# scroll-tech/zkevm-circuits

Hardware: AMD Instinct MI355X
Metric: SuperCircuit-shape proof-gen wall-clock (s) at k = 20 (lower is better)
Workload: dtype u32x8 limbs (254-bit modular integer, Montgomery)

## Files before the change

### zkevm-circuits_amd/csrc/msm.hip

```cpp
#include <chrono>
#include <climits>
#include <cmath>

#include "ctx.hpp"
#include "ec29.hip.hpp"
#include "host_fq.hpp"

namespace zk {

constexpr int MSM_MAX_C = 16;
constexpr uint32_t NEG_BIT = 0x80000000u;

struct MsmPlan {
    int c;
    int W;
    uint32_t B;
    int top_shift = 0;
};

struct MsmCol { const Fr* scalars; G1Xyzz* out; };

static MsmPlan make_plan(size_t n) {
    int lg = 0;
    while ((1ull << (lg + 1)) <= n) ++lg;
// ... 141 lines not shown
    uint32_t carry = 0;
#pragma unroll
    for (int w = 0; w < W; ++w) {
        const int bit = w * C, limb = bit >> 5, sh = bit & 31;
        uint32_t d = limb < 8 ? (s.l[limb < 8 ? limb : 7] >> sh) : 0u;
        if (sh + C > 32 && limb + 1 < 8) d |= s.l[limb + 1 < 8 ? limb + 1 : 7] << (32 - sh);
        d = (d & mask) + carry;
        if (w == W - 1) d <<= top_shift;
        if (d > half) { carry = 1; const uint32_t mag = (1u << C) - d; code[w] = mag ? (NEG_BIT | (mag - 1)) : CODE_ZERO; }
        else { carry = 0; code[w] = d ? (d - 1) : CODE_ZERO; }
    }
}
__device__ __forceinline__ uint32_t lds_take(uint32_t* lds, uint32_t slot, bool active) {
    const uint64_t act = __ballot(active);
    if (!active) return 0;
    const uint32_t lane = threadIdx.x & 63u;
    const uint32_t lead = __shfl(slot, (int)__builtin_ctzll(act));
    const uint64_t same = __ballot(slot == lead);
    if (slot == lead) {
        const uint32_t rank = (uint32_t)__popcll(same & ((1ull << lane) - 1ull));
        uint32_t pos = 0;
        if (rank == 0) pos = atomicAdd(&lds[slot], (uint32_t)__popcll(same));
        return __shfl(pos, (int)__builtin_ctzll(same)) + rank;
    }
    return atomicAdd(&lds[slot], 1u);
}
template <int C, bool SCATTER, bool LOWPART = false>
__device__ __forceinline__ void partition_body(const Fr* __restrict__ scalars, uint64_t n, int range_bits, uint32_t* __restrict__ hist, const uint32_t* __restrict__ hist_off,
                                               uint64_t* __restrict__ entries, uint64_t tab_stride, int top_shift, uint32_t bin_base, uint32_t set_mask, uint32_t nwg, uint32_t g, uint32_t* lds) {
    constexpr int W = (256 + C - 1) / C;
    const uint32_t nbins = (set_mask + 1u) << (C - 1 - range_bits);
    for (uint32_t t = threadIdx.x; t < nbins; t += blockDim.x) lds[t] = SCATTER ? hist_off[(uint64_t)(bin_base + t) * nwg + g] : 0u;
    __syncthreads();
    const uint64_t chunk = (n + nwg - 1) / nwg;
    const uint64_t lo = min(n, (uint64_t)g * chunk), hi = min(n, lo + chunk);
    const uint32_t rmask = (1u << range_bits) - 1u;
    for (uint64_t base = lo; base < hi; base += blockDim.x) {
        const uint64_t i = base + threadIdx.x;
        const bool live = i < hi;
        uint32_t code[W];
        if (live) recode_wide<C>(from_mont(ldg(scalars + i)), code, top_shift);
        else {
#pragma unroll
            for (int w = 0; w < W; ++w) code[w] = CODE_ZERO;
        }
#pragma unroll
        for (int w = 0; w < W; ++w) {
            const bool nz = code[w] != CODE_ZERO;
            if (!__ballot(nz)) continue;
            uint32_t part, local;
            if (LOWPART) {
                const int PB = C - 1 - range_bits;
                const uint32_t b = code[w] & 0x3FFFFFu;
                part = ((((uint32_t)w & set_mask)) << PB) | (b & ((1u << PB) - 1u));
                local = b >> PB;
            } else {
                const uint32_t bucket = (code[w] & 0x3FFFFFu) | (((uint32_t)w & set_mask) << (C - 1));
                part = bucket >> range_bits;
                local = bucket & rmask;
            }
            const uint32_t pos = lds_take(lds, part, nz);
            if (SCATTER && nz) entries[pos] = ((uint64_t)local << 32) | (uint64_t)((uint32_t)((uint64_t)w * tab_stride + i) | (code[w] & NEG_BIT));
        }
    }
    if (!SCATTER) {
        __syncthreads();
        for (uint32_t t = threadIdx.x; t < nbins; t += blockDim.x) hist[(uint64_t)(bin_base + t) * nwg + g] = lds[t];
    }
}
template <int C, bool SCATTER>
__global__ void __launch_bounds__(256) k_msm_m_partition(const Fr* __restrict__ scalars_arg, uint64_t n, int range_bits, uint32_t* __restrict__ hist, const uint32_t* __restrict__ hist_off,
                                                          uint64_t* __restrict__ entries, uint64_t tab_stride, int top_shift, const MsmCol* __restrict__ cols = nullptr, const uint32_t* __restrict__ ctr = nullptr) {
    const Fr* __restrict__ scalars = cols ? cols[*ctr].scalars : scalars_arg;
    __shared__ uint32_t lds[MSM_M_MAX_BINS];
    partition_body<C, SCATTER>(scalars, n, range_bits, hist, hist_off, entries, tab_stride, top_shift, 0u, 0u, gridDim.x, blockIdx.x, lds);
}
constexpr int GM_MAX_COLS = 16;
struct GmCols { const Fr* p[GM_MAX_COLS]; };
template <int C, bool SCATTER>
__global__ void __launch_bounds__(256) k_msm_gm_partition(GmCols cols, uint64_t n, int range_bits, uint32_t* __restrict__ hist, const uint32_t* __restrict__ hist_off,
                                                           uint64_t* __restrict__ entries, uint64_t tab_stride, uint32_t bins_per_col, uint32_t set_mask) {
    __shared__ uint32_t lds[MSM_M_MAX_BINS];
    partition_body<C, SCATTER, true>(cols.p[blockIdx.y], n, range_bits, hist, hist_off, entries, tab_stride, 0, blockIdx.y * bins_per_col, set_mask, gridDim.x, blockIdx.x, lds);
}
constexpr uint32_t MSM_M_SCHUNK = 1024;
template <int C>
__global__ void __launch_bounds__(1024) k_msm_m_scatter_staged(const Fr* __restrict__ scalars_arg, uint64_t n, int range_bits, const uint32_t* __restrict__ hist_off,
                                                               uint64_t* __restrict__ entries, uint64_t tab_stride, int top_shift, const MsmCol* __restrict__ cols = nullptr, const uint32_t* __restrict__ ctr = nullptr) {
    constexpr int W = (256 + C - 1) / C;
    const Fr* __restrict__ scalars = cols ? cols[*ctr].scalars : scalars_arg;
    extern __shared__ __attribute__((aligned(16))) uint32_t sm[];
    uint32_t* cnt = sm;
    uint32_t* gdelta = sm + MSM_M_MAX_BINS;
    uint32_t* wtot = gdelta + MSM_M_MAX_BINS;
    uint64_t* stage = reinterpret_cast<uint64_t*>(wtot + 16);
    uint16_t* pid = reinterpret_cast<uint16_t*>(stage + (size_t)MSM_M_SCHUNK * W);
    const uint32_t nbins = 1u << (C - 1 - range_bits), nwg = gridDim.x, g = blockIdx.x;
    const uint32_t rmask = (1u << range_bits) - 1u;
    cnt[threadIdx.x] = 0u;
    __syncthreads();
    const uint64_t chunk = (n + nwg - 1) / nwg;
    const uint64_t i = min(n, (uint64_t)g * chunk) + threadIdx.x;
    const bool live = threadIdx.x < chunk && i < min(n, ((uint64_t)g + 1) * chunk);
    uint32_t code[W], rank[W];
    if (live) recode_wide<C>(from_mont(ldg(scalars + i)), code, top_shift);
    else {
#pragma unroll
        for (int w = 0; w < W; ++w) code[w] = CODE_ZERO;
    }
#pragma unroll
    for (int w = 0; w < W; ++w) {
        const bool nz = code[w] != CODE_ZERO;
        rank[w] = 0;
        if (!__ballot(nz)) continue;
        rank[w] = lds_take(cnt, (code[w] & 0x3FFFFFu) >> range_bits, nz);
    }
    __syncthreads();
    {
        const uint32_t c0 = threadIdx.x < nbins ? cnt[threadIdx.x] : 0u;
        const uint32_t lane = threadIdx.x & 63u, wave = threadIdx.x >> 6;
        uint32_t incl = c0;
#pragma unroll
        for (int off = 1; off < 64; off <<= 1) { const uint32_t o = __shfl_up(incl, off); if (lane >= (uint32_t)off) incl += o; }
        if (lane == 63) wtot[wave] = incl;
        __syncthreads();
        uint32_t wbase = 0;
        for (uint32_t w = 0; w < wave; ++w) wbase += wtot[w];
        const uint32_t ex = wbase + incl - c0;
        if (threadIdx.x < nbins) {
            cnt[threadIdx.x] = ex;
            gdelta[threadIdx.x] = hist_off[(uint64_t)threadIdx.x * nwg + g] - ex;
        }
    }
    __syncthreads();
    uint32_t total = 0;
    for (uint32_t w = 0; w < 16; ++w) total += wtot[w];
#pragma unroll
    for (int w = 0; w < W; ++w) {
        if (code[w] == CODE_ZERO) continue;
        const uint32_t bucket = code[w] & 0x3FFFFFu, part = bucket >> range_bits;
        const uint32_t pos = cnt[part] + rank[w];
        stage[pos] = ((uint64_t)(bucket & rmask) << 32) | (uint64_t)((uint32_t)((uint64_t)w * tab_stride + i) | (code[w] & NEG_BIT));
        pid[pos] = (uint16_t)part;
    }
    __syncthreads();
    for (uint32_t e = threadIdx.x; e < total; e += blockDim.x) entries[gdelta[pid[e]] + e] = stage[e];
}
static size_t scatter_staged_lds(int W) { return (size_t)(2 * MSM_M_MAX_BINS + 16) * 4 + (size_t)MSM_M_SCHUNK * W * 10; }
template <bool SCATTER>
__global__ void __launch_bounds__(1024) k_msm_m_bin(const uint64_t* __restrict__ entries, const uint32_t* __restrict__ hist_off, uint32_t nwg, int range_bits,
                                                    uint32_t* __restrict__ counts, const uint32_t* __restrict__ offsets, uint32_t* __restrict__ idx) {
    __shared__ uint32_t lds[1 << MSM_RANGE_MAX_BITS];
    const uint32_t nbins_ = gridDim.x / MSM_SLICES;
    uint32_t bin, sl;
    if ((nbins_ & 7u) == 0) {
        const uint32_t xcd = blockIdx.x & 7u, slot = blockIdx.x >> 3;
        sl = slot % MSM_SLICES;
        bin = (slot / MSM_SLICES) * 8u + xcd;
    } else {
        bin = blockIdx.x / MSM_SLICES;
        sl = blockIdx.x % MSM_SLICES;
    }
    const uint32_t range = 1u << range_bits;
    const uint64_t gbase = (uint64_t)bin << range_bits;
    for (uint32_t t = threadIdx.x; t < range; t += blockDim.x) lds[t] = SCATTER ? offsets[(gbase + t) * MSM_SLICES + sl] : 0u;
    __syncthreads();
// ... 570 lines not shown
    __syncthreads();
}
template <bool LAST>
__global__ void __launch_bounds__(256) k_wsum_level(const G1Xyzz29* __restrict__ in, uint32_t count, G1Xyzz29* __restrict__ S_out, G1Xyzz29* __restrict__ Tpart, G1Xyzz29* __restrict__ U_out) {
    __shared__ G1Xyzz29 sh[LAST ? 512 : 256];
    const uint32_t g = blockIdx.x * 256 + threadIdx.x, groups = (count + WS_G - 1) / WS_G;
    G1Xyzz29 acc = identity29(), run = identity29();
    if (g < groups) {
        const uint32_t b0 = g * WS_G, b1 = min(b0 + WS_G, count);
        for (uint32_t b = b1; b-- > b0;) { acc = add29pt(acc, run); run = add29pt(run, ldg29(in + b)); }
        if (LAST) { if (b0) acc = add29pt(acc, mul_small(run, b0)); }
        else stg29(S_out + g, run);
    }
    if (LAST) {
        block_sum29x2(acc, run, sh);
        if (threadIdx.x == 0) { stg29(Tpart + blockIdx.x, acc); stg29(U_out, run); }
    } else {
        const G1Xyzz29 t = block_sum29(acc, sh);
        if (threadIdx.x == 0) stg29(Tpart + blockIdx.x, t);
    }
}
struct WsumPlan { int levels; uint32_t off[WS_MAX_LEVELS], cnt[WS_MAX_LEVELS]; };
__global__ void __launch_bounds__(256) k_wsum_final(const G1Xyzz29* __restrict__ Tpart, WsumPlan pl, const G1Xyzz29* __restrict__ U, G1Xyzz* __restrict__ out) {
    __shared__ G1Xyzz29 A[WS_MAX_LEVELS];
    const uint32_t wave = threadIdx.x >> 6, lane = threadIdx.x & 63u;
    for (int lv = (int)wave; lv < pl.levels; lv += 4) {
        G1Xyzz29 a = identity29();
        for (uint32_t i = lane; i < pl.cnt[lv]; i += 64) a = add29pt(a, ldg29(Tpart + pl.off[lv] + i));
        for (int off = 32; off > 0; off >>= 1) a = add29pt(a, shfl_down_pt(a, off));
        if (lane == 0) A[lv] = a;
    }
    __syncthreads();
    if (threadIdx.x == 0) {
        G1Xyzz29 T = A[pl.levels - 1];
        for (int lv = pl.levels - 2; lv >= 0; --lv) {
            for (int d = 1; d < WS_G; d <<= 1) T = dbl29pt(T);
            T = add29pt(T, A[lv]);
        }
        stg(out, to_std_xyzz(add29pt(T, ldg29(U))));
    }
}
static int wsum_enqueue(zk_ctx* ctx, hipStream_t st, const G1Xyzz29* buckets, uint32_t nb, G1Xyzz29* scratch, G1Xyzz* out) {
    WsumPlan pl;
    pl.levels = 0;
    uint32_t tparts = 0, count = nb;
    uint32_t t_total = 1;
    for (uint32_t c_ = nb; ; ) {
        const uint32_t groups = (c_ + WS_G - 1) / WS_G;
        t_total += c_ <= WS_LAST_MAX ? 1 : (groups + 255) / 256;
        if (c_ <= WS_LAST_MAX) break;
        c_ = groups;
    }
    G1Xyzz29* U = scratch;
    G1Xyzz29* Tpart = scratch + 1;
    G1Xyzz29* S = scratch + t_total;
    const G1Xyzz29* in = buckets;
    while (count > WS_LAST_MAX) {
        if (pl.levels >= WS_MAX_LEVELS - 1) return ctx->fail(ZK_ERR_UNSUPPORTED, "bucket reduction: too many levels");
        const uint32_t groups = (count + WS_G - 1) / WS_G, blocks = (groups + 255) / 256;
        pl.off[pl.levels] = tparts; pl.cnt[pl.levels] = blocks;
        hipLaunchKernelGGL((k_wsum_level<false>), dim3(blocks), dim3(256), 0, st, in, count, S, Tpart + tparts, (G1Xyzz29*)nullptr);
        tparts += blocks;
        ++pl.levels;
        in = S;
        S += groups;
        count = groups;
    }
    pl.off[pl.levels] = tparts; pl.cnt[pl.levels] = 1;
    hipLaunchKernelGGL((k_wsum_level<true>), dim3(1), dim3(256), 0, st, in, count, (G1Xyzz29*)nullptr, Tpart + tparts, U);
    ++pl.levels;
    hipLaunchKernelGGL(k_wsum_final, dim3(1), dim3(256), 0, st, (const G1Xyzz29*)Tpart, pl, (const G1Xyzz29*)U, out);
    ZK_CHECK_LAUNCH(ctx);
    return ZK_OK;
}

#define PK_TRY_MSM(expr) do { int rc__ = (expr); if (rc__) return rc__; } while (0)

constexpr int KNOB_UNSET = INT_MIN;
struct MsmKnobs {
    int c, top_shift;
    int binsort, staged, chunk;
    int pipes, graph;
    int narrow, narrow_group, narrow_gm, gm_sets;
    double table_gb;
    bool trace;
};
static MsmKnobs read_knobs() {
    auto num = [](const char* name) { const char* e = getenv(name); return e ? atoi(e) : KNOB_UNSET; };
    MsmKnobs k;
    k.c = num("ZK_MSM_C");
    k.top_shift = num("ZK_MSM_TOP_SHIFT");
    k.binsort = num("ZK_MSM_BINSORT");
    k.staged = num("ZK_MSM_STAGED");
    k.chunk = num("ZK_MSM_CHUNK");
    k.pipes = num("ZK_MSM_PIPES");
    k.graph = num("ZK_MSM_GRAPH");
    k.narrow = num("ZK_MSM_NARROW");
    k.narrow_group = num("ZK_MSM_NARROW_GROUP");
    k.narrow_gm = num("ZK_MSM_NARROW_GM");
    k.gm_sets = num("ZK_MSM_GM_SETS");
    const char* gb = getenv("ZK_MSM_TABLE_GB");
    k.table_gb = gb ? atof(gb) : 32.0;
    k.trace = getenv("ZK_MSM_TRACE") != nullptr;
    return k;
}

struct WsCarver {
    uint32_t* base;
    size_t at = 0;
    uint32_t* take(size_t nwords, size_t align_words = 1) {
        at = (at + align_words - 1) / align_words * align_words;
        uint32_t* p = base ? base + at : nullptr;
        at += nwords;
        return p;
    }
};
static inline uint32_t scan_blocks_of(uint32_t cnt) { return (cnt + SCAN_T * SCAN_ITEMS - 1) / (SCAN_T * SCAN_ITEMS); }
constexpr uint32_t MSM_CLEARED_WORDS = SIZE_BINS + 4 + MSM_WFLAGS + TASK_DONE_MAX;
struct SortDims {
    uint32_t nb;
    bool slices;
    uint32_t hist_cnt;
    uint64_t idx_cnt;
    size_t dig_words;
    bool entries;
};
struct SortWs {
    uint32_t *slice_counts, *slice_off, *block_tot_s;
    uint32_t *counts, *offsets, *order, *ntasks, *toff, *block_tot;
    uint32_t *cleared, *size_hist, *nmulti, *wflag;
    uint32_t *hist, *hist_off, *block_tot_h;
    uint32_t* idx;
    uint16_t* dig;
    uint64_t* entries;
    size_t words;
};
static SortWs carve_sort_ws(const SortDims& d, uint32_t* base) {
    WsCarver c{base};
    SortWs w{};
    if (d.slices) {
        w.slice_counts = c.take((size_t)d.nb * MSM_SLICES, 4);
        w.slice_off = c.take((size_t)d.nb * MSM_SLICES + 4, 4);
    }
    w.counts = c.take(d.nb);
    w.cleared = c.take(MSM_CLEARED_WORDS);
    w.size_hist = w.cleared;
    w.nmulti = w.size_hist + SIZE_BINS;
    w.wflag = w.nmulti + 4;
    w.offsets = c.take((size_t)d.nb + 1);
    w.order = c.take(d.nb);
    w.ntasks = c.take(d.nb);
    w.toff = c.take((size_t)d.nb + 1);
    if (d.slices) w.block_tot_s = c.take(scan_blocks_of(d.nb * MSM_SLICES));
    w.block_tot = c.take(scan_blocks_of(d.nb));
    if (d.hist_cnt) {
        w.block_tot_h = c.take(scan_blocks_of(d.hist_cnt));
        w.hist = c.take(d.hist_cnt);
        w.hist_off = c.take((size_t)d.hist_cnt + 1);
    }
    w.idx = c.take(d.idx_cnt);
    if (d.dig_words) w.dig = reinterpret_cast<uint16_t*>(c.take(d.dig_words, 4));
    if (d.entries) w.entries = reinterpret_cast<uint64_t*>(c.take(2 * (size_t)d.idx_cnt, 2));
    w.words = c.at;
    return w;
}

static void scan_blocks(hipStream_t st, const uint32_t* in, uint32_t cnt, uint32_t* out, uint32_t* block_tot, uint32_t* total_out) {
    const uint32_t sb = scan_blocks_of(cnt);
    hipLaunchKernelGGL(k_scan_u32_a, dim3(sb), dim3(SCAN_T), 0, st, in, cnt, out, block_tot);
    hipLaunchKernelGGL(k_scan_u32_b, dim3(1), dim3(SCAN_T), 0, st, block_tot, sb, out, cnt, total_out);
}
static int exclusive_scan(zk_ctx* ctx, hipStream_t st, const uint32_t* in, uint32_t cnt, uint32_t* out, uint32_t* block_tot) {
    scan_blocks(st, in, cnt, out, block_tot, nullptr);
    hipLaunchKernelGGL(k_task_offsets, dim3(scan_blocks_of(cnt)), dim3(SCAN_T), 0, st, cnt, out, (const uint32_t*)block_tot);
    ZK_CHECK_LAUNCH(ctx);
    return ZK_OK;
}
static int slice_scan(zk_ctx* ctx, hipStream_t st, const SortWs& w, uint32_t nb) {
    scan_blocks(st, w.slice_counts, nb * MSM_SLICES, w.slice_off, w.block_tot_s, w.offsets + nb);
    hipLaunchKernelGGL(k_scan_u32_c, dim3(scan_blocks_of(nb * MSM_SLICES)), dim3(SCAN_T), 0, st, (const uint32_t*)w.slice_counts, nb, w.slice_off, (const uint32_t*)w.block_tot_s, w.offsets, w.counts,
                       w.size_hist);
    ZK_CHECK_LAUNCH(ctx);
    return ZK_OK;
// ... 118 lines not shown
    ZK_HIP(ctx, hipEventRecord(ctx->ev_p2[par], ctx->stream2));
    if (stage && it + 1 < count) { int rc = stage(stage_user, it + 1); if (rc) return rc; }
  }
    ZK_HIP(ctx, hipStreamWaitEvent(ctx->stream, ctx->ev_p2[0], 0));
    if (count > 1) ZK_HIP(ctx, hipStreamWaitEvent(ctx->stream, ctx->ev_p2[1], 0));
    std::vector<G1Xyzz> hw((size_t)pl.W * count);
    ZK_HIP(ctx, hipMemcpyAsync(hw.data(), wsum_all, sizeof(G1Xyzz) * pl.W * count, hipMemcpyDeviceToHost, ctx->stream));
    ZK_HIP(ctx, hipStreamSynchronize(ctx->stream));
    for (size_t it = 0; it < count; ++it) host::msm_tail(hw.data() + it * pl.W, red_W, pl.c, h_out + it);
    return ZK_OK;
}
__global__ void __launch_bounds__(1024) k_msm_tails(const Fr* const* __restrict__ scalar_ptrs, const uint8_t* __restrict__ flags, uint64_t n_main, uint32_t tail,
                                                    const G1Affine* __restrict__ table, uint64_t tab_stride, int c, int W, int top_shift, G1Xyzz* __restrict__ out) {
    __shared__ G1Xyzz29 wsum[16];
    const uint32_t col = blockIdx.x;
    G1Xyzz29 acc = identity29();
    if (flags[col] == 1) {
        const Fr* scalars = scalar_ptrs[col];
        for (uint32_t pair = threadIdx.x; pair < tail * (uint32_t)W; pair += blockDim.x) {
            const uint32_t r = pair / (uint32_t)W, w = pair % (uint32_t)W;
            const Fr sc = from_mont(ldg(scalars + n_main + r));
            const int bit = (int)w * c, limb = bit >> 5, sh = bit & 31;
            uint64_t d = limb < 8 ? ((uint64_t)sc.l[limb] >> sh) : 0ull;
            if (limb + 1 < 8) d |= (uint64_t)sc.l[limb + 1] << (32 - sh);
            d &= (1ull << c) - 1;
            int bits = c;
            if ((int)w == W - 1) { d <<= top_shift; bits = c + top_shift; }
            if (d == 0) continue;
            const G1Affine29 base = load_affine29(table + (uint64_t)w * tab_stride + n_main + r);
            G1Xyzz29 t = identity29();
            for (int b = bits - 1; b >= 0; --b) {
                t = dbl29pt(t);
                if ((d >> b) & 1) t = madd29(t, base);
            }
            acc = add29pt(acc, t);
        }
    }
    for (int off = 32; off > 0; off >>= 1) acc = add29pt(acc, shfl_down_pt(acc, off));
    if ((threadIdx.x & 63) == 0) wsum[threadIdx.x >> 6] = acc;
    __syncthreads();
    if (threadIdx.x == 0) {
        G1Xyzz29 s = wsum[0];
        for (uint32_t i = 1; i < blockDim.x / 64; ++i) s = add29pt(s, wsum[i]);
        stg(out + col, to_std_xyzz(s));
    }
}
static MsmPlan make_plan_merged(uint32_t k_srs, const MsmKnobs& kn) {
    int c = (int)k_srs;
    if (c < MSM_M_MIN_C) c = MSM_M_MIN_C;
    if (c > MSM_M_MAX_C) c = MSM_M_MAX_C;
    if (kn.c >= MSM_M_MIN_C && kn.c <= MSM_M_MAX_C) c = kn.c;
    MsmPlan p;
    p.c = c;
    p.W = (256 + c - 1) / c;
    p.B = 1u << (c - 1);
    const int low = c * (p.W - 1);
    uint64_t top_max = 1;
    if (low < 254) {
        uint64_t v = 0;
        for (int b = 0; b < 40 && low + b < 256; ++b) {
            const int bit = low + b;
            const uint32_t limb = bit < 32 ? FrP::M(0) - 1u : FrP::M(bit >> 5);
            v |= (uint64_t)((limb >> (bit & 31)) & 1u) << b;
        }
        top_max = v + 1;
    }
    p.top_shift = 0;
    while (p.top_shift + 1 <= c - 1 && (top_max << (p.top_shift + 1)) <= (1ull << (c - 1))) ++p.top_shift;
    if (kn.top_shift >= 0 && kn.top_shift <= p.top_shift) p.top_shift = kn.top_shift;
    return p;
}
template <bool SCATTER>
static void launch_partition(int c, dim3 grid, hipStream_t st, const Fr* scalars, uint64_t n, int range_bits, uint32_t* hist, const uint32_t* hist_off, uint64_t* entries, uint64_t tab_stride, int top_shift,
                             const MsmCol* cols = nullptr, const uint32_t* ctr = nullptr) {
#define ZK_PART_CASE(C) case C: hipLaunchKernelGGL((k_msm_m_partition<C, SCATTER>), grid, dim3(256), 0, st, scalars, n, range_bits, hist, hist_off, entries, tab_stride, top_shift, cols, ctr); break;
    switch (c) {
        ZK_PART_CASE(8) ZK_PART_CASE(9) ZK_PART_CASE(10) ZK_PART_CASE(11) ZK_PART_CASE(12) ZK_PART_CASE(13) ZK_PART_CASE(14) ZK_PART_CASE(15)
        ZK_PART_CASE(16) ZK_PART_CASE(17) ZK_PART_CASE(18) ZK_PART_CASE(19) ZK_PART_CASE(20) ZK_PART_CASE(21) ZK_PART_CASE(22)
    }
#undef ZK_PART_CASE
}
template <bool SCATTER>
static void launch_gm_partition(int c, dim3 grid, hipStream_t st, const GmCols& cols, uint64_t n, int range_bits, uint32_t* hist, const uint32_t* hist_off, uint64_t* entries, uint64_t tab_stride,
                                uint32_t bins_per_col, uint32_t set_mask) {
#define ZK_GMP_CASE(C) case C: hipLaunchKernelGGL((k_msm_gm_partition<C, SCATTER>), grid, dim3(256), 0, st, cols, n, range_bits, hist, hist_off, entries, tab_stride, bins_per_col, set_mask); break;
    switch (c) {
        ZK_GMP_CASE(8) ZK_GMP_CASE(9) ZK_GMP_CASE(10) ZK_GMP_CASE(11) ZK_GMP_CASE(12) ZK_GMP_CASE(13) ZK_GMP_CASE(14) ZK_GMP_CASE(15) ZK_GMP_CASE(16)
    }
#undef ZK_GMP_CASE
}
static int launch_scatter_staged(zk_ctx* ctx, int c, int W, dim3 grid, const Fr* scalars, uint64_t n, int range_bits, const uint32_t* hist_off, uint64_t* entries, uint64_t tab_stride, int top_shift,
                                 const MsmCol* cols = nullptr, const uint32_t* ctr = nullptr, hipStream_t st = nullptr) {
    const size_t lds = scatter_staged_lds(W);
    if (!st) st = ctx->stream;
#define ZK_SS_CASE(C) case C: \
        if (!(ctx->msm_attr_set & (1u << C))) { ZK_HIP(ctx, hipFuncSetAttribute((const void*)k_msm_m_scatter_staged<C>, hipFuncAttributeMaxDynamicSharedMemorySize, (int)lds)); ctx->msm_attr_set |= 1u << C; } \
        hipLaunchKernelGGL((k_msm_m_scatter_staged<C>), grid, dim3(1024), lds, st, scalars, n, range_bits, hist_off, entries, tab_stride, top_shift, cols, ctr); break;
    switch (c) { ZK_SS_CASE(19) ZK_SS_CASE(20) ZK_SS_CASE(21) ZK_SS_CASE(22) default: return ctx->fail(ZK_ERR_UNSUPPORTED, "staged scatter: window size %d", c); }
#undef ZK_SS_CASE
    ZK_CHECK_LAUNCH(ctx);
    return ZK_OK;
}
static int sort_entries(zk_ctx* ctx, hipStream_t st, const SortWs& w, uint32_t nbins, uint32_t nwg, int range_bits, uint32_t nb, bool binsort) {
    if (binsort) {
        hipLaunchKernelGGL(k_msm_m_binsort, dim3(nbins), dim3(1024), 0, st, (const uint64_t*)w.entries, (const uint32_t*)w.hist_off, nwg, range_bits, nb, w.offsets, w.counts, w.size_hist, w.idx);
        ZK_CHECK_LAUNCH(ctx);
        return task_split(ctx, st, w, nb);
    }
    hipLaunchKernelGGL((k_msm_m_bin<false>), dim3(nbins * MSM_SLICES), dim3(1024), 0, st, (const uint64_t*)w.entries, (const uint32_t*)w.hist_off, nwg, range_bits, w.slice_counts, (const uint32_t*)nullptr, (uint32_t*)nullptr);
    ZK_CHECK_LAUNCH(ctx);
    PK_TRY_MSM(slice_scan(ctx, st, w, nb));
    PK_TRY_MSM(task_split(ctx, st, w, nb));
    hipLaunchKernelGGL((k_msm_m_bin<true>), dim3(nbins * MSM_SLICES), dim3(1024), 0, st, (const uint64_t*)w.entries, (const uint32_t*)w.hist_off, nwg, range_bits, (uint32_t*)nullptr, (const uint32_t*)w.slice_off, w.idx);
    ZK_CHECK_LAUNCH(ctx);
    return ZK_OK;
}
static int sort_partitioned(zk_ctx* ctx, hipStream_t st, const SortWs& w, const MsmPlan& pl, const Fr* scalars, uint64_t n, uint64_t tab_stride, int range_bits, uint32_t nwg, bool staged_scatter, bool binsort,
                            const MsmCol* cols, const uint32_t* ctr) {
    const uint32_t nbins = pl.B >> range_bits;
    ZK_HIP(ctx, hipMemsetAsync(w.cleared, 0, (size_t)MSM_CLEARED_WORDS * 4, st));
    launch_partition<false>(pl.c, dim3(nwg), st, scalars, n, range_bits, w.hist, (const uint32_t*)nullptr, (uint64_t*)nullptr, tab_stride, pl.top_shift, cols, ctr);
    ZK_CHECK_LAUNCH(ctx);
    PK_TRY_MSM(exclusive_scan(ctx, st, w.hist, nbins * nwg, w.hist_off, w.block_tot_h));
    if (staged_scatter) PK_TRY_MSM(launch_scatter_staged(ctx, pl.c, pl.W, dim3(nwg), scalars, n, range_bits, (const uint32_t*)w.hist_off, w.entries, tab_stride, pl.top_shift, cols, ctr, st));
    else launch_partition<true>(pl.c, dim3(nwg), st, scalars, n, range_bits, (uint32_t*)nullptr, (const uint32_t*)w.hist_off, w.entries, tab_stride, pl.top_shift, cols, ctr);
    ZK_CHECK_LAUNCH(ctx);
    return sort_entries(ctx, st, w, nbins, nwg, range_bits, pl.B, binsort);
}
static int sort_gm(zk_ctx* ctx, hipStream_t st, const SortWs& w, const MsmPlan& pl, const Fr* const* scalars, uint32_t cnt, uint64_t n, uint64_t tab_stride, int range_bits, uint32_t nwg, uint32_t bpc, uint32_t sets) {
    const uint32_t nbins = cnt * bpc;
    ZK_HIP(ctx, hipMemsetAsync(w.cleared, 0, (size_t)MSM_CLEARED_WORDS * 4, st));
    GmCols gcols{};
    for (uint32_t j = 0; j < cnt; ++j) gcols.p[j] = scalars[j];
    launch_gm_partition<false>(pl.c, dim3(nwg, cnt), st, gcols, n, range_bits, w.hist, (const uint32_t*)nullptr, (uint64_t*)nullptr, tab_stride, bpc, sets - 1);
    ZK_CHECK_LAUNCH(ctx);
    PK_TRY_MSM(exclusive_scan(ctx, st, w.hist, nbins * nwg, w.hist_off, w.block_tot_h));
    launch_gm_partition<true>(pl.c, dim3(nwg, cnt), st, gcols, n, range_bits, (uint32_t*)nullptr, (const uint32_t*)w.hist_off, w.entries, tab_stride, bpc, sets - 1);
    ZK_CHECK_LAUNCH(ctx);
    return sort_entries(ctx, st, w, nbins, nwg, range_bits, cnt * sets * pl.B, true);
}
static int msm_batch_merged_capped(zk_ctx* ctx, const MsmKnobs& kn, const Fr* const* d_scalar_ptrs, size_t count, const G1Affine* d_table, size_t tab_stride, const MsmPlan& pl,
                                   size_t n, G1Affine* h_out, MsmStageFn stage, void* stage_user, const G1Affine* d_table_n, const MsmPlan* pl_n, const uint8_t* narrow, uint32_t group_cap, uint32_t* smaller_cap) {
    if (count == 0) return ZK_OK;
    if (n == 0) { memset(h_out, 0, sizeof(G1Affine) * count); return ZK_OK; }
    const auto t_batch0 = std::chrono::steady_clock::now();
    bool any_narrow = false;
    if (d_table_n && pl_n && narrow) for (size_t i = 0; i < count; ++i) any_narrow |= narrow[i] == 1;
    if (any_narrow && (uint64_t)n * pl_n->W >= (1ull << 32)) any_narrow = false;
    const uint32_t tail_rows = (any_narrow && ctx->msm_blinded_tail && (size_t)ctx->msm_blinded_tail + 1024 <= n && ctx->msm_blinded_tail <= 256) ? ctx->msm_blinded_tail : 0u;
    const uint64_t n_narrow = (uint64_t)n - tail_rows;
    const MsmPlan pn = any_narrow ? *pl_n : MsmPlan{4, 64, 8};
    uint32_t NG = 1;
    if (any_narrow) {
        NG = std::min<uint32_t>((uint32_t)GM_MAX_COLS, MSM_WFLAGS / (uint32_t)pn.W);
        if (kn.narrow_group >= 1 && kn.narrow_group <= GM_MAX_COLS) NG = std::min<uint32_t>((uint32_t)kn.narrow_group, MSM_WFLAGS / (uint32_t)pn.W);
        if (group_cap && NG > group_cap) NG = group_cap;
        while (NG > 1 && (uint64_t)n * pn.W * NG >= (1ull << 32)) --NG;
        if (NG < 1) NG = 1;
    }
    const uint32_t Wg = (uint32_t)pn.W * NG;
    const uint32_t nbN = Wg * pn.B;
    const uint64_t n_pad = ((uint64_t)n + 16 * MSM_SLICES - 1) & ~(uint64_t)(16 * MSM_SLICES - 1);
    const SortDims dims_N{nbN, true, 0, (uint64_t)n * Wg, (size_t)(n_pad * Wg + 1) / 2 + 4, false};
    const bool gm = any_narrow && pn.c >= MSM_M_MIN_C && pn.c <= 16 && NG <= (uint32_t)GM_MAX_COLS && kn.narrow_gm != 0;
    uint32_t SG = 2;
    if (kn.gm_sets == 1 || kn.gm_sets == 2 || kn.gm_sets == 4) SG = (uint32_t)kn.gm_sets;
    int range_bits_G = pn.c - 1 - 7;
    if (range_bits_G < 0) range_bits_G = 0;
    const uint32_t bpcG = (SG * pn.B) >> range_bits_G;
    const uint32_t perm_G = ((uint32_t)range_bits_G << 8) | (uint32_t)(pn.c - 1 - range_bits_G);
    const uint32_t nwgG = (uint32_t)((n_narrow + MSM_M_CHUNK - 1) / MSM_M_CHUNK);
    const SortDims dims_G{NG * SG * pn.B, false, NG * bpcG * nwgG, (uint64_t)n * pn.W * NG, 0, true};
    const size_t words_N = any_narrow ? std::max(carve_sort_ws(dims_N, nullptr).words, gm ? carve_sort_ws(dims_G, nullptr).words : 0) : 0;
    const uint32_t red_blocks_N = ((pn.B + RED_G_WIDE - 1) / RED_G_WIDE + RED_THREADS - 1) / RED_THREADS;
    const size_t max_tasks_N = (size_t)nbN + std::max(((size_t)n * Wg) / TASK_CAP, (size_t)TASK_TARGET) + 1;
    const size_t npts29_N = any_narrow ? (size_t)nbN + (size_t)red_blocks_N * NG * 4 + max_tasks_N + (size_t)pn.B * NG : 0;
    const uint32_t nb = pl.B;
    const uint64_t max_entries = (uint64_t)n * pl.W;
    if ((uint64_t)pl.W * tab_stride >= (1ull << 31) || max_entries >= (1ull << 32)) return ctx->fail(ZK_ERR_UNSUPPORTED, "MSM of %zu points x %d windows exceeds the 32-bit entry space: split it", n, pl.W);
    int range_bits = pl.c - 1;
    if (range_bits > MSM_RANGE_MAX_BITS) range_bits = MSM_RANGE_MAX_BITS;
    bool binsort = kn.binsort != 0;
    if (binsort) {
        int rb = pl.c - 1 - 10;
        if (rb < 0) rb = 0;
        const uint64_t per_partition = max_entries / (nb >> rb);
        if (per_partition + per_partition / 8 <= MSM_M_STAGE) range_bits = rb;
        else binsort = false;
    }
    uint32_t chunk = MSM_M_CHUNK;
    if (kn.chunk >= 256 && kn.chunk <= 65536) chunk = (uint32_t)kn.chunk;
    const bool staged_scatter = binsort && pl.c >= 19 && scatter_staged_lds(pl.W) <= (size_t)150 * 1024 && kn.staged != 0;
    if (staged_scatter) chunk = MSM_M_SCHUNK;
    const uint32_t nwg = (uint32_t)((n + chunk - 1) / chunk);
    const SortDims dims_M{nb, true, (nb >> range_bits) * nwg, max_entries, 0, true};
    const size_t words_M = carve_sort_ws(dims_M, nullptr).words;
    const size_t words = (std::max(words_M, words_N) + 63) & ~(size_t)63;
    int npipe = (n <= ((size_t)1 << 19) && count >= 2) ? 2 : 1;
    if (kn.pipes == 1 || (kn.pipes == 2 && count >= 2)) npipe = kn.pipes;
    const bool want_graph = n <= ((size_t)1 << 19) && n >= 1024 && count >= 4 && !ctx->prof_on && !ctx->msm_graph_broken && kn.graph != 0 && !(any_narrow && NG > 1);
    constexpr int GP = 4;
    uint32_t* ws = (uint32_t*)ctx->get_scratch(SC_MSM_KEYS, words * 4 * (want_graph ? GP : npipe));
    if (!ws && any_narrow && NG > 1 && words_N > words_M) {
        (void)hipGetLastError();
        *smaller_cap = NG / 2;
        return ZK_ERR_OOM;
    }
    if (!ws) return ZK_ERR_OOM;
    const uint32_t red_pts = nb / 4 + 1024;
    const size_t max_tasks = (size_t)nb + std::max((size_t)(max_entries / TASK_CAP), (size_t)TASK_TARGET) + 1;
    const size_t npts29 = std::max((size_t)nb + red_pts + max_tasks, npts29_N);
    char* bkbuf[3];
    bkbuf[0] = (char*)ctx->get_scratch(SC_MSM_BUCKETS, sizeof(G1Xyzz29) * npts29);
    bkbuf[1] = count > 1 ? (char*)ctx->get_scratch(SC_MSM_BUCKETS2, sizeof(G1Xyzz29) * npts29) : bkbuf[0];
    bkbuf[2] = count > 2 ? (char*)ctx->get_scratch(SC_MSM_BUCKETS3, sizeof(G1Xyzz29) * npts29) : bkbuf[0];
    G1Xyzz* wsum_all = (G1Xyzz*)ctx->get_scratch(SC_MSM_RESULTS, sizeof(G1Xyzz) * count + 4 * MSM_WFLAGS * count);
    if (!bkbuf[0] || !bkbuf[1] || !bkbuf[2] || !wsum_all) return ZK_ERR_OOM;
    if (!ctx->stream2) ZK_HIP(ctx, hipStreamCreateWithFlags(&ctx->stream2, hipStreamNonBlocking));
    if (!ctx->ev_p1[0])
        for (int i = 0; i < 3; ++i) {
// ... 83 lines not shown
                                                     (uint64_t)(uintptr_t)ws, (uint64_t)words, (uint64_t)(uintptr_t)bk[p], (uint64_t)(uintptr_t)desc, (uint64_t)staged_scatter, (uint64_t)range_bits, n_narrow,
                                                     (uint64_t)pl.top_shift, (uint64_t)nwg};
            uint64_t key = 1469598103934665603ull;
            for (uint64_t v : key_tuple) key = (key ^ v) * 1099511628211ull;
            hipGraphExec_t exec = nullptr;
            auto found = ctx->msm_graphs.find(key);
            if (found != ctx->msm_graphs.end() && ctx->msm_graph_keys[key] != key_tuple) {
                (void)hipGraphExecDestroy((hipGraphExec_t)found->second);
                ctx->msm_graphs.erase(found);
                found = ctx->msm_graphs.end();
            }
            if (found != ctx->msm_graphs.end()) exec = (hipGraphExec_t)found->second;
            else {
                if (ctx->msm_graphs.size() >= 48) {
                    ZK_HIP(ctx, hipStreamSynchronize(P[0]));
                    for (int q = 1; q < GP; ++q) ZK_HIP(ctx, hipStreamSynchronize(P[q]));
                    for (auto& kv : ctx->msm_graphs) (void)hipGraphExecDestroy((hipGraphExec_t)kv.second);
                    ctx->msm_graphs.clear();
                    ctx->msm_graph_keys.clear();
                }
                hipGraph_t graph = nullptr;
                bool ok = hipStreamBeginCapture(P[p], hipStreamCaptureModeRelaxed) == hipSuccess;
                int rc_e = ok ? enqueue(kind, p) : ZK_ERR_HIP;
                if (ok) ok = hipStreamEndCapture(P[p], &graph) == hipSuccess && graph != nullptr;
                ok = ok && rc_e == ZK_OK && hipGraphInstantiate(&exec, graph, nullptr, nullptr, 0) == hipSuccess;
                if (graph) (void)hipGraphDestroy(graph);
                if (!ok) {
                    const hipError_t e = hipGetLastError();
                    if (kn.trace) fprintf(stderr, "[zk msm] graph capture failed (rc %d, %s): plain launches from now on\n", rc_e, hipGetErrorString(e));
                    ctx->msm_graph_broken = true; fallback = true; break;
                }
                ctx->msm_graphs[key] = (void*)exec;
                ctx->msm_graph_keys[key] = key_tuple;
            }
            if (hipGraphLaunch(exec, P[p]) != hipSuccess) {
                const hipError_t e = hipGetLastError();
                if (kn.trace) fprintf(stderr, "[zk msm] graph replay failed (%s): plain launches from now on\n", hipGetErrorString(e));
                ctx->msm_graph_broken = true; fallback = true; break;
            }
            if (stage && it + 1 < count) { ctx->stream = P[(it + 1) % GP]; int rc = stage(stage_user, it + 1); if (rc) return rc; }
        }
        ctx->stream = P[0];
        for (int p = 1; p < GP; ++p) {
            ZK_HIP(ctx, hipEventRecord(ctx->ev_p2[p - 1], P[p]));
            ZK_HIP(ctx, hipStreamWaitEvent(P[0], ctx->ev_p2[p - 1], 0));
        }
        if (!fallback) return finish(" (graph replay)");
        ZK_HIP(ctx, hipStreamSynchronize(ctx->stream));
    }
    hipStream_t mains[2] = {ctx->stream, npipe == 2 ? ctx->stream2c : ctx->stream};
    struct StreamRestore { zk_ctx* c; hipStream_t s; ~StreamRestore() { c->stream = s; } } restore{ctx, ctx->stream};
    if (npipe == 2) {
        ZK_HIP(ctx, hipEventRecord(ctx->ev_pipe, mains[0]));
        ZK_HIP(ctx, hipStreamWaitEvent(mains[1], ctx->ev_pipe, 0));
    }
    auto is_narrow = [&](size_t it) { return any_narrow && narrow[it] == 1; };
    auto group_of = [&](size_t it) -> size_t {
        if (!is_narrow(it)) return 1;
        size_t g = 1;
        while (g < NG && it + g < count && is_narrow(it + g)) ++g;
        return g;
    };
    if (stage) { int rc = stage(stage_user, 0); if (rc) return rc; }
    size_t staged = stage ? 1 : count;
    size_t stepno = 0;
    for (size_t it = 0; it < count; ++stepno) {
        const size_t grp = group_of(it);
        const int par = (int)(stepno % 3), pipe = (int)(stepno % (size_t)npipe);
        hipStream_t side = npipe == 2 ? ((stepno & 1) ? ctx->stream2b : ctx->stream2) : (par == 0 ? ctx->stream2 : par == 1 ? ctx->stream2b : ctx->stream2c);
        ctx->stream = mains[pipe];
        for (; staged < it + grp; ++staged) { int rc = stage(stage_user, staged); if (rc) return rc; }
        const bool nar = is_narrow(it), grouped = nar && gm;
        const uint32_t cnt = (uint32_t)grp;
        const uint32_t nbc = grouped ? cnt * SG * pn.B : nar ? cnt * (uint32_t)pn.W * pn.B : nb;
        const size_t tasks = nar ? (size_t)nbc + std::max(((size_t)n * cnt * pn.W) / TASK_CAP, (size_t)TASK_TARGET) + 1 : max_tasks;
        const SortWs w = carve_sort_ws(grouped ? dims_G : nar ? dims_N : dims_M, ws + (size_t)pipe * words);
        uint32_t* wflag_it = reinterpret_cast<uint32_t*>(wsum_all + count) + it * MSM_WFLAGS;
        G1Xyzz29* buckets = (G1Xyzz29*)bkbuf[par];
        G1Xyzz29* partial = buckets + (nar ? nbN : nb);
        G1Xyzz29* task_partial = partial + (grouped ? (size_t)red_blocks_N * NG * 4 : nar ? (size_t)red_blocks_N * NG : red_pts);
        G1Xyzz29* folded = task_partial + max_tasks_N;
        {
            ZkProfScope ps(ctx, "msm_sort");
            if (grouped) PK_TRY_MSM(sort_gm(ctx, ctx->stream, w, pn, d_scalar_ptrs + it, cnt, n_narrow, (uint64_t)tab_stride, range_bits_G, nwgG, bpcG, SG));
            else if (nar) {
                PK_TRY_MSM(sort_digits(ctx, ctx->stream, w, pn, d_scalar_ptrs + it, cnt, n_narrow, n_pad, nullptr, nullptr));
                ZK_HIP(ctx, hipMemcpyAsync(wflag_it, w.wflag, MSM_WFLAGS * sizeof(uint32_t), hipMemcpyDeviceToDevice, ctx->stream));
            } else {
                PK_TRY_MSM(sort_partitioned(ctx, ctx->stream, w, pl, d_scalar_ptrs[it], (uint64_t)n, (uint64_t)tab_stride, range_bits, nwg, staged_scatter, binsort && !(narrow && narrow[it] == 2), nullptr, nullptr));
            }
        }
        if (stepno >= 3) ZK_HIP(ctx, hipStreamWaitEvent(ctx->stream, ctx->ev_p2[par], 0));
        if (grouped) PK_TRY_MSM(accumulate_combine(ctx, ctx->stream, "msm_buckets_narrow", d_table_n, w, nbc, tasks, buckets, task_partial, 0, 0, nullptr, 0, perm_G));
        else if (nar) PK_TRY_MSM(accumulate_combine(ctx, ctx->stream, "msm_buckets_narrow", d_table_n, w, nbc, tasks, buckets, task_partial, pn.c - 1, (uint64_t)tab_stride, wflag_it, cnt > 1 ? (uint32_t)pn.W : 0u, 0));
        else PK_TRY_MSM(accumulate_combine(ctx, ctx->stream, "msm_buckets", d_table, w, nb, tasks, buckets, task_partial, 0, 0, nullptr, 0, 0));
        ZK_HIP(ctx, hipEventRecord(ctx->ev_p1[par], ctx->stream));
        ZK_HIP(ctx, hipStreamWaitEvent(side, ctx->ev_p1[par], 0));
        {
            ZkProfScope ps(ctx, nar ? "msm_reduce_narrow" : "msm_reduce", side);
            if (grouped) PK_TRY_MSM(reduce_window(ctx, side, buckets, pn.B, 0, nullptr, nullptr, cnt, SG, false, partial, wsum_all + it, nullptr, nullptr, 0));
            else if (nar) PK_TRY_MSM(reduce_window(ctx, side, buckets, pn.B, pn.W, folded, wflag_it, cnt, 1, false, partial, wsum_all + it, nullptr, nullptr, 0));
            else if (it + 2 >= count) PK_TRY_MSM(reduce_window(ctx, side, buckets, nb, 0, nullptr, nullptr, 1, 1, false, partial, wsum_all + it, nullptr, nullptr, 0));
            else PK_TRY_MSM(wsum_enqueue(ctx, side, buckets, nb, partial, wsum_all + it));
        }
        ZK_HIP(ctx, hipEventRecord(ctx->ev_p2[par], side));
        if (stage && it + grp < count) {
            ctx->stream = mains[(stepno + 1) % (size_t)npipe];
            const size_t upto = it + grp + group_of(it + grp);
            for (; staged < upto; ++staged) { int rc = stage(stage_user, staged); if (rc) return rc; }
        }
        it += grp;
    }
    ctx->stream = mains[0];
    if (npipe == 2) {
        ZK_HIP(ctx, hipEventRecord(ctx->ev_pipe, mains[1]));
        ZK_HIP(ctx, hipStreamWaitEvent(mains[0], ctx->ev_pipe, 0));
    }
    ZK_HIP(ctx, hipStreamWaitEvent(ctx->stream, ctx->ev_p2[0], 0));
    if (stepno > 1) ZK_HIP(ctx, hipStreamWaitEvent(ctx->stream, ctx->ev_p2[1], 0));
    if (stepno > 2) ZK_HIP(ctx, hipStreamWaitEvent(ctx->stream, ctx->ev_p2[2], 0));
    return finish("");
}
int msm_batch_merged(zk_ctx* ctx, const MsmKnobs& kn, const Fr* const* d_scalar_ptrs, size_t count, const G1Affine* d_table, size_t tab_stride, const MsmPlan& pl,
                     size_t n, G1Affine* h_out, MsmStageFn stage, void* stage_user, const G1Affine* d_table_n = nullptr, const MsmPlan* pl_n = nullptr, const uint8_t* narrow = nullptr) {
    for (uint32_t cap = 0;;) {
        uint32_t smaller_cap = 0;
        const int rc = msm_batch_merged_capped(ctx, kn, d_scalar_ptrs, count, d_table, tab_stride, pl, n, h_out, stage, stage_user, d_table_n, pl_n, narrow, cap, &smaller_cap);
        if (!smaller_cap) return rc;
        cap = smaller_cap;
    }
}
static int srs_window_table_narrow(zk_ctx* ctx, const zk_srs* srs, int basis, size_t n, const G1Affine** out, MsmPlan* plan) {
    *out = nullptr;
    zk_srs* s = const_cast<zk_srs*>(srs);
    const uint64_t ns = 1ull << s->k;
    const MsmPlan pl = make_plan(ns);
    *plan = pl;
    const size_t bytes = sizeof(G1Affine) * ns * pl.W;
    const double cap_gb = read_knobs().table_gb;
    if (n < 1024 || (double)bytes > cap_gb * (double)(1ull << 30)) return ZK_OK;
    if (!s->tabn[basis]) {
        const G1Affine* rp = nullptr;
        int rc = srs_bases_rp(ctx, srs, basis, &rp);
        if (rc) return rc;
        if (hipMalloc(&s->tabn[basis], bytes) != hipSuccess) { (void)hipGetLastError(); s->tabn[basis] = nullptr; return ZK_OK; }
        hipLaunchKernelGGL(k_build_window_tables, dim3((unsigned)((ns + 255) / 256)), dim3(256), 0, ctx->stream, rp, ns, pl.c, pl.W, s->tabn[basis], 0);
        ZK_CHECK_LAUNCH(ctx);
    }
    *out = s->tabn[basis];
    return ZK_OK;
}
int msm_batch_srs(zk_ctx* ctx, const zk_srs* srs, int basis, const Fr* const* d_scalar_ptrs, size_t count, size_t n, G1Affine* h_out, MsmStageFn stage, void* stage_user, const uint8_t* narrow) {
    static thread_local bool runs_tried = false;
    if (narrow && !stage && count && !runs_tried) {
        bool any2 = false;
        for (size_t i = 0; i < count; ++i) any2 |= narrow[i] == 2;
        if (any2) {
            std::vector<uint8_t> done(count);
            int rc = msm_runs_try(ctx, srs, basis, d_scalar_ptrs, count, n, narrow, h_out, done.data());
            if (rc) return rc;
            std::vector<size_t> rest;
            for (size_t i = 0; i < count; ++i) if (!done[i]) rest.push_back(i);
            if (rest.size() < count) {
                if (rest.empty()) return ZK_OK;
                std::vector<const Fr*> ptrs(rest.size());
                std::vector<uint8_t> hints(rest.size());
                std::vector<G1Affine> outs(rest.size());
// ... 235 lines not shown
```

Before: 1.897.

## Add dense wave-compacted partition kernel for grouped narrow MSM columns

Adds a grouped-MSM partition kernel that compacts nonzero scalars within each wavefront through LDS stacks, then compacts nonzero digit records, so that recoding and bin updates run on full waves. It is meant to avoid wasting lanes on zero scalars and zero digits in sparse narrow columns. The kernel is selected unless ZK_MSM_GM_DENSE=0 and only when bins per column fit in 512. The cost is extra LDS traffic, wave-level bookkeeping, and more register and LDS pressure.

```diff
diff --git a/zkevm-circuits_amd/csrc/msm.hip b/zkevm-circuits_amd/csrc/msm.hip
--- a/zkevm-circuits_amd/csrc/msm.hip
+++ b/zkevm-circuits_amd/csrc/msm.hip
@@ -247,6 +247,112 @@
                                                            uint64_t* __restrict__ entries, uint64_t tab_stride, uint32_t bins_per_col, uint32_t set_mask) {
     __shared__ uint32_t lds[MSM_M_MAX_BINS];
     partition_body<C, SCATTER, true>(cols.p[blockIdx.y], n, range_bits, hist, hist_off, entries, tab_stride, 0, blockIdx.y * bins_per_col, set_mask, gridDim.x, blockIdx.x, lds);
+}
+constexpr uint32_t GM_DENSE_MAX_BINS = 512;
+struct GmWaveStacks {
+    uint4 cell_lo[64], cell_hi[64];
+    uint64_t rec[64];
+    uint32_t row[64];
+};
+template <bool SCATTER>
+__device__ __forceinline__ void gm_dense_take(uint32_t* bins, uint64_t rec, bool active, uint64_t* __restrict__ entries) {
+    const uint32_t pos = lds_take(bins, (uint32_t)(rec >> 48), active);
+    if (SCATTER && active) entries[pos] = rec & 0x0000FFFFFFFFFFFFull;
+}
+template <int C, bool SCATTER>
+__device__ __forceinline__ void gm_dense_recode(uint32_t* bins, GmWaveStacks& q, const uint4& a, const uint4& b, uint32_t row, bool active, uint32_t& len_r, int PB, uint32_t set_mask,
+                                                uint64_t tab_stride, uint64_t* __restrict__ entries, uint64_t lt) {
+    constexpr int W = (256 + C - 1) / C;
+    uint32_t code[W];
+    if (active) {
+        Fr s;
+        s.l[0] = a.x; s.l[1] = a.y; s.l[2] = a.z; s.l[3] = a.w; s.l[4] = b.x; s.l[5] = b.y; s.l[6] = b.z; s.l[7] = b.w;
+        recode_wide<C>(from_mont(s), code, 0);
+    } else {
+#pragma unroll
+        for (int w = 0; w < W; ++w) code[w] = CODE_ZERO;
+    }
+#pragma unroll
+    for (int w = 0; w < W; ++w) {
+        const bool nz = code[w] != CODE_ZERO;
+        const uint64_t m = __ballot(nz);
+        if (!m) continue;
+        const uint32_t bk = code[w] & 0x3FFFFFu;
+        const uint32_t part = (((uint32_t)w & set_mask) << PB) | (bk & ((1u << PB) - 1u)), local = bk >> PB;
+        const uint32_t payload = (uint32_t)((uint64_t)w * tab_stride + row) | (code[w] & NEG_BIT);
+        uint64_t rec = ((uint64_t)((part << 16) | local) << 32) | payload;
+        const uint32_t have = (uint32_t)__popcll(m), holes = 64u - have;
+        if (len_r >= holes) {
+            if (!nz) rec = q.rec[len_r - 1u - (uint32_t)__popcll(~m & lt)];
+            len_r = __builtin_amdgcn_readfirstlane(len_r - holes);
+            gm_dense_take<SCATTER>(bins, rec, true, entries);
+        } else {
+            if (nz) q.rec[len_r + (uint32_t)__popcll(m & lt)] = rec;
+            len_r = __builtin_amdgcn_readfirstlane(len_r + have);
+        }
+        __builtin_amdgcn_fence(__ATOMIC_ACQ_REL, "wavefront");
+    }
+}
+template <int C, bool SCATTER>
+__global__ void __launch_bounds__(256) k_msm_gm_partition_dense(GmCols cols, uint64_t n, int range_bits, uint32_t* __restrict__ hist, const uint32_t* __restrict__ hist_off,
+                                                                 uint64_t* __restrict__ entries, uint64_t tab_stride, uint32_t bins_per_col, uint32_t set_mask) {
+    __shared__ uint32_t bins[GM_DENSE_MAX_BINS];
+    __shared__ GmWaveStacks stacks[4];
+    const Fr* __restrict__ scalars = cols.p[blockIdx.y];
+    const uint32_t nwg = gridDim.x, g = blockIdx.x, bin_base = blockIdx.y * bins_per_col;
+    const int PB = C - 1 - range_bits;
+    const uint32_t nbins = (set_mask + 1u) << PB;
+    for (uint32_t t = threadIdx.x; t < nbins; t += blockDim.x) bins[t] = SCATTER ? hist_off[(uint64_t)(bin_base + t) * nwg + g] : 0u;
+    __syncthreads();
+    const uint64_t chunk = (n + nwg - 1) / nwg;
+    const uint64_t lo = min(n, (uint64_t)g * chunk), hi = min(n, lo + chunk);
+    GmWaveStacks& q = stacks[threadIdx.x >> 6];
+    const uint32_t lane = threadIdx.x & 63u;
+    const uint64_t lt = (1ull << lane) - 1ull;
+    uint32_t len_c = 0, len_r = 0;
+    const uint64_t last = n - 1;
+    const uint4* p0 = reinterpret_cast<const uint4*>(scalars + min(lo + threadIdx.x, last));
+    uint4 an = p0[0], bn = p0[1];
+    for (uint64_t base = lo; base < hi; base += blockDim.x) {
+        const uint64_t i = base + threadIdx.x, inext = i + blockDim.x;
+        uint4 a = an, b = bn;
+        const uint4* pn = reinterpret_cast<const uint4*>(scalars + min(inext, last));
+        an = pn[0]; bn = pn[1];
+        const bool nzc = i < hi && ((a.x | a.y | a.z | a.w) | (b.x | b.y | b.z | b.w)) != 0u;
+        const uint64_t m = __ballot(nzc);
+        const uint32_t have = (uint32_t)__popcll(m), holes = 64u - have;
+        if (len_c >= holes) {
+            uint32_t row = (uint32_t)i;
+            if (!nzc) {
+                const uint32_t slot = len_c - 1u - (uint32_t)__popcll(~m & lt);
+                a = q.cell_lo[slot]; b = q.cell_hi[slot]; row = q.row[slot];
+            }
+            len_c = __builtin_amdgcn_readfirstlane(len_c - holes);
+            __builtin_amdgcn_fence(__ATOMIC_ACQ_REL, "wavefront");
+            gm_dense_recode<C, SCATTER>(bins, q, a, b, row, true, len_r, PB, set_mask, tab_stride, entries, lt);
+        } else {
+            if (nzc) {
+                const uint32_t slot = len_c + (uint32_t)__popcll(m & lt);
+                q.cell_lo[slot] = a; q.cell_hi[slot] = b; q.row[slot] = (uint32_t)i;
+            }
+            len_c = __builtin_amdgcn_readfirstlane(len_c + have);
+            __builtin_amdgcn_fence(__ATOMIC_ACQ_REL, "wavefront");
+        }
+    }
+    if (len_c) {
+        uint4 a = make_uint4(0, 0, 0, 0), b = a;
+        uint32_t row = 0;
+        if (lane < len_c) { a = q.cell_lo[lane]; b = q.cell_hi[lane]; row = q.row[lane]; }
+        gm_dense_recode<C, SCATTER>(bins, q, a, b, row, lane < len_c, len_r, PB, set_mask, tab_stride, entries, lt);
+    }
+    if (len_r) {
+        const uint64_t rec = lane < len_r ? q.rec[lane] : 0ull;
+        gm_dense_take<SCATTER>(bins, rec, lane < len_r, entries);
+    }
+    if (!SCATTER) {
+        __syncthreads();
+        for (uint32_t t = threadIdx.x; t < nbins; t += blockDim.x) hist[(uint64_t)(bin_base + t) * nwg + g] = bins[t];
+    }
 }
 constexpr uint32_t MSM_M_SCHUNK = 1024;
 template <int C>
@@ -983,6 +1089,7 @@
     int binsort, staged, chunk;
     int pipes, graph;
     int narrow, narrow_group, narrow_gm, gm_sets;
+    int gm_dense;
     double table_gb;
     bool trace;
 };
@@ -1000,6 +1107,7 @@
     k.narrow_group = num("ZK_MSM_NARROW_GROUP");
     k.narrow_gm = num("ZK_MSM_NARROW_GM");
     k.gm_sets = num("ZK_MSM_GM_SETS");
+    k.gm_dense = num("ZK_MSM_GM_DENSE");
     const char* gb = getenv("ZK_MSM_TABLE_GB");
     k.table_gb = gb ? atof(gb) : 32.0;
     k.trace = getenv("ZK_MSM_TRACE") != nullptr;
@@ -1284,8 +1392,11 @@
 }
 template <bool SCATTER>
 static void launch_gm_partition(int c, dim3 grid, hipStream_t st, const GmCols& cols, uint64_t n, int range_bits, uint32_t* hist, const uint32_t* hist_off, uint64_t* entries, uint64_t tab_stride,
-                                uint32_t bins_per_col, uint32_t set_mask) {
-#define ZK_GMP_CASE(C) case C: hipLaunchKernelGGL((k_msm_gm_partition<C, SCATTER>), grid, dim3(256), 0, st, cols, n, range_bits, hist, hist_off, entries, tab_stride, bins_per_col, set_mask); break;
+                                uint32_t bins_per_col, uint32_t set_mask, bool dense) {
+#define ZK_GMP_CASE(C) case C: \
+        if (dense) hipLaunchKernelGGL((k_msm_gm_partition_dense<C, SCATTER>), grid, dim3(256), 0, st, cols, n, range_bits, hist, hist_off, entries, tab_stride, bins_per_col, set_mask); \
+        else hipLaunchKernelGGL((k_msm_gm_partition<C, SCATTER>), grid, dim3(256), 0, st, cols, n, range_bits, hist, hist_off, entries, tab_stride, bins_per_col, set_mask); \
+        break;
     switch (c) {
         ZK_GMP_CASE(8) ZK_GMP_CASE(9) ZK_GMP_CASE(10) ZK_GMP_CASE(11) ZK_GMP_CASE(12) ZK_GMP_CASE(13) ZK_GMP_CASE(14) ZK_GMP_CASE(15) ZK_GMP_CASE(16)
     }
@@ -1329,15 +1440,17 @@
     ZK_CHECK_LAUNCH(ctx);
     return sort_entries(ctx, st, w, nbins, nwg, range_bits, pl.B, binsort);
 }
-static int sort_gm(zk_ctx* ctx, hipStream_t st, const SortWs& w, const MsmPlan& pl, const Fr* const* scalars, uint32_t cnt, uint64_t n, uint64_t tab_stride, int range_bits, uint32_t nwg, uint32_t bpc, uint32_t sets) {
+static int sort_gm(zk_ctx* ctx, hipStream_t st, const SortWs& w, const MsmPlan& pl, const Fr* const* scalars, uint32_t cnt, uint64_t n, uint64_t tab_stride, int range_bits, uint32_t nwg, uint32_t bpc, uint32_t sets,
+                   bool dense) {
     const uint32_t nbins = cnt * bpc;
+    dense = dense && bpc <= GM_DENSE_MAX_BINS;
     ZK_HIP(ctx, hipMemsetAsync(w.cleared, 0, (size_t)MSM_CLEARED_WORDS * 4, st));
     GmCols gcols{};
     for (uint32_t j = 0; j < cnt; ++j) gcols.p[j] = scalars[j];
-    launch_gm_partition<false>(pl.c, dim3(nwg, cnt), st, gcols, n, range_bits, w.hist, (const uint32_t*)nullptr, (uint64_t*)nullptr, tab_stride, bpc, sets - 1);
+    launch_gm_partition<false>(pl.c, dim3(nwg, cnt), st, gcols, n, range_bits, w.hist, (const uint32_t*)nullptr, (uint64_t*)nullptr, tab_stride, bpc, sets - 1, dense);
     ZK_CHECK_LAUNCH(ctx);
     PK_TRY_MSM(exclusive_scan(ctx, st, w.hist, nbins * nwg, w.hist_off, w.block_tot_h));
-    launch_gm_partition<true>(pl.c, dim3(nwg, cnt), st, gcols, n, range_bits, (uint32_t*)nullptr, (const uint32_t*)w.hist_off, w.entries, tab_stride, bpc, sets - 1);
+    launch_gm_partition<true>(pl.c, dim3(nwg, cnt), st, gcols, n, range_bits, (uint32_t*)nullptr, (const uint32_t*)w.hist_off, w.entries, tab_stride, bpc, sets - 1, dense);
     ZK_CHECK_LAUNCH(ctx);
     return sort_entries(ctx, st, w, nbins, nwg, range_bits, cnt * sets * pl.B, true);
 }
@@ -1587,7 +1700,7 @@
         G1Xyzz29* folded = task_partial + max_tasks_N;
         {
             ZkProfScope ps(ctx, "msm_sort");
-            if (grouped) PK_TRY_MSM(sort_gm(ctx, ctx->stream, w, pn, d_scalar_ptrs + it, cnt, n_narrow, (uint64_t)tab_stride, range_bits_G, nwgG, bpcG, SG));
+            if (grouped) PK_TRY_MSM(sort_gm(ctx, ctx->stream, w, pn, d_scalar_ptrs + it, cnt, n_narrow, (uint64_t)tab_stride, range_bits_G, nwgG, bpcG, SG, kn.gm_dense != 0));
             else if (nar) {
                 PK_TRY_MSM(sort_digits(ctx, ctx->stream, w, pn, d_scalar_ptrs + it, cnt, n_narrow, n_pad, nullptr, nullptr));
                 ZK_HIP(ctx, hipMemcpyAsync(wflag_it, w.wflag, MSM_WFLAGS * sizeof(uint32_t), hipMemcpyDeviceToDevice, ctx->stream));
```

Result: no change. 1.883 (median of 6 runs) (-0.7%).
